# GT-RIPL/robo-vln

Measured on AMD Instinct MI355X. Metric: policy env-steps/sec (batched act()) at 256x256 RGB-D, 80-tok instr, higher is better.
Workload: dtype fp16 (range-calibrated fp16 storage and MFMA in BERT, both trunks and the cross-modal block; fp32 accumulate, fp32 recurrent state; DESIGN.md section 5); 1 GPU; BASELINE.json configs[1]: full HCM act() (hi->argmax->lo), 256x256 RGB-D, L=80, VLA N=1, LSTM-512; per_gpu_batch=64, global_batch=64, parallelism=single GPU

## Files before the change

### include/hcm.h

```cpp
#ifndef HCM_H
#define HCM_H

#include <stdint.h>

#ifdef __cplusplus
extern "C" {
#endif

typedef struct hcm_ctx* hcm_handle;

enum hcm_status {
    HCM_OK = 0,
    HCM_ERR_ARG = -1,
    HCM_ERR_STATE = -2,
    HCM_ERR_KEY = -3,
    HCM_ERR_SHAPE = -4,
    HCM_ERR_HIP = -5,
    HCM_ERR_UNSUPPORTED = -6,
    HCM_ERR_NOMEM = -7
};

enum hcm_dtype { HCM_F32 = 0, HCM_BF16 = 1, HCM_I32 = 2, HCM_I64 = 3, HCM_U8 = 4, HCM_F16 = 5 };
enum hcm_model { HCM_HIGH = 0, HCM_LOW = 1, HCM_CMA = 2 ,
                 HCM_S2S = 3  };
// ... 173 lines not shown
                  int act, void* stream);
int hcm_op_conv2d_gn(const void* x, const void* w_ohwi, const float* gamma, const float* beta, const void* residual, void* y,
                     int dtype, int B, int H, int W, int Cin, int Cout, int KH, int KW, int stride, int pad, int groups, float eps,
                     int relu, void* stream);
int hcm_op_bottleneck_tail(const void* x, const void* w2, const float* b2, const void* w3, const float* b3, const void* identity,
                           void* y, int dtype, int B, int H, int W, int C1, int stride, void* stream);
int hcm_op_bottleneck_tail_next(const void* x, const void* w2, const float* b2, const void* w3, const float* b3, const void* identity,
                                void* y, const void* w1, const float* b1, void* o1, int dtype, int B, int H, int W, int C1, int stride,
                                int CN, void* stream);
int hcm_op_bottleneck_tail_ds(const void* x, const void* w2, const float* b2, const void* w3ds, const float* b3ds, const void* xd,
                              void* y, const void* w1, const float* b1, void* o1, int dtype, int B, int H, int W, int stride,
                              void* stream);
int hcm_op_conv2d_gn_large(const void* x, const void* w_ohwi, const float* gamma, const float* beta, const void* residual, void* y,
                           int dtype, int B, int H, int W, int Cin, int Cout, int KH, int KW, int stride, int pad, int groups, float eps,
                           int relu, void* stream);
int hcm_op_stem_conv(const void* x, int x_dtype, const void* w, const float* bias, void* y, int dtype, int B, int H, int W, int C,
                     int Cout, int KH, int KW, int stride, int pad, int K, int Kp, int rowrun, float scale, int act, void* stream);
int hcm_op_stem_conv_packed(const void* x, int x_dtype, const void* w, const float* bias, void* y, int dtype, int B, int H, int W,
                            int Cout, float scale, int act, void* scratch, void* stream);
int hcm_op_stem_conv_packed_pool(const void* x, int x_dtype, const void* w, const float* bias, void* y, int dtype, int B, int H, int W,
                                 int Cout, float scale, void* scratch, void* half_map, void* stream);
int hcm_op_stem_pool_fused(const void* x, int x_dtype, const void* w, const float* bias, void* y, int dtype, int B, int H, int W,
                           int Cout, float scale, void* scratch, void* stream);
int hcm_op_stem_pool_fused_red(const void* x, int x_dtype, const void* w, const float* bias, void* y, int dtype, int B, int H, int W,
                               int Cout, float scale, void* scratch, const void* w1, const float* b1, void* o1, void* stream);
int64_t hcm_op_stem_scratch_bytes(int B, int H, int W);
int hcm_op_depth_conv8x8s4(const float* depth, const void* w, const float* bias, void* y, int dtype, int B, int H, int act, void* scratch,
                           void* stream);
int hcm_op_simplecnn3(const float* depth, const void* w0, const float* b0, const void* w1_frag, const float* b1, const void* w2_frag, const float* b2,
                      void* y, int dtype, int B, int H, void* stream);
// ... 37 lines not shown
```

### robo-vln_amd/_lib.py

```python
import ctypes as C
import os

_HERE = os.path.dirname(os.path.abspath(__file__))
LIB_PATH = os.path.join(_HERE, "libhcm_dev.so" if os.environ.get("HCM_DEV_LIB", "0") not in ("", "0") else "libhcm.so")

HCM_F32, HCM_BF16, HCM_I32, HCM_I64, HCM_U8, HCM_F16 = 0, 1, 2, 3, 4, 5
HCM_HIGH, HCM_LOW, HCM_CMA, HCM_S2S = 0, 1, 2, 3
HCM_ENC_RESNET, HCM_ENC_SIMPLECNN = 0, 1
HCM_LSTM, HCM_GRU = 0, 1
(HCM_NUM_RECURRENT_LAYERS, HCM_HIDDEN_SIZE, HCM_NUM_ACTIONS, HCM_RECORD_WIDTH, HCM_WORKSPACE_BYTES,
 HCM_WEIGHT_BYTES, HCM_MAX_BATCH, HCM_GRAPH_LAUNCHES, HCM_EAGER_LAUNCHES, HCM_FP16_FALLBACK, HCM_CALIB_MAX_BERT, HCM_CALIB_MAX_DEPTH,
 HCM_CALIB_NONFINITE, HCM_CALIB_MAX_RGB, HCM_CALIB_MAX_VLA, HCM_STEP_NONFINITE, HCM_RANGE_FOLD, HCM_GATHER_JOINED) = range(18)
PRECISIONS = {"fp32": HCM_F32, "fp16": HCM_F16, "bf16": HCM_BF16}
ACT_NONE, ACT_RELU, ACT_GELU = 0, 1, 2
HCM_ACT_REUSE_INSTRUCTION = 1
HCM_ACT_HOST_FRAMES = 2
HCM_ACT_CHAIN_GRAPHS = 4

STATUS_EXC = {-1: ValueError, -2: RuntimeError, -3: KeyError, -4: ValueError, -5: RuntimeError, -6: ValueError,
              -7: MemoryError}


class HcmConfigStruct(C.Structure):
    _fields_ = [(n, C.c_int32) for n in (
# ... 78 lines not shown
    "hcm_op_stem_pool_fused_red": (C.c_int, [C.c_void_p, C.c_int, C.c_void_p, C.c_void_p, C.c_void_p] + [C.c_int] * 5 + [C.c_float] + [C.c_void_p] * 5),
    "hcm_op_stem_conv_packed_pool": (C.c_int, [C.c_void_p, C.c_int, C.c_void_p, C.c_void_p, C.c_void_p] + [C.c_int] * 5 + [C.c_float, C.c_void_p, C.c_void_p, C.c_void_p]),
    "hcm_op_depth_conv8x8s4": (C.c_int, [C.c_void_p] * 4 + [C.c_int] * 4 + [C.c_void_p, C.c_void_p]),
    "hcm_op_stem_scratch_bytes": (C.c_int64, [C.c_int] * 3),
    "hcm_op_linear": (C.c_int, [C.c_void_p] * 5 + [C.c_int] * 6 + [C.c_void_p]),
    "hcm_op_linear_impl": (C.c_int, [C.c_void_p] * 5 + [C.c_int] * 7 + [C.c_void_p]),
    "hcm_op_vla_layer": (C.c_int, [C.c_void_p] * 7 + [C.c_int] + [C.c_void_p] * 11 + [C.c_int] * 5 + [C.c_void_p]),
    "hcm_op_vla_layer_frag": (C.c_int, [C.c_void_p] * 7 + [C.c_int] + [C.c_void_p] * 11 + [C.c_int] * 5 + [C.c_void_p]),
    "hcm_op_attention": (C.c_int, [C.c_void_p] * 4 + [C.c_int] * 9 + [C.c_void_p]),
    "hcm_op_simplecnn3": (C.c_int, [C.c_void_p] * 8 + [C.c_int] * 3 + [C.c_void_p]),
    "hcm_op_pack_frag": (C.c_int, [C.c_void_p, C.c_void_p, C.c_int, C.c_int, C.c_int, C.c_void_p]),
    "hcm_op_bert_attn_block": (C.c_int, [C.c_void_p] * 9 + [C.c_int] * 3 + [C.c_void_p, C.c_float, C.c_void_p]),
    "hcm_op_layernorm": (C.c_int, [C.c_void_p] * 5 + [C.c_int] * 3 + [C.c_float, C.c_void_p]),
    "hcm_op_layernorm_post": (C.c_int, [C.c_void_p] * 5 + [C.c_int, C.c_void_p] + [C.c_int] * 3 + [C.c_float, C.c_void_p]),
    "hcm_op_groupnorm": (C.c_int, [C.c_void_p] * 4 + [C.c_int] * 5 + [C.c_float, C.c_int, C.c_void_p]),
    "hcm_op_conv2d_gn_pool": (C.c_int, [C.c_void_p] * 5 + [C.c_int] * 11 + [C.c_float, C.c_void_p]),
    "hcm_op_conv2d_gn_res2": (C.c_int, [C.c_void_p] * 9 + [C.c_int] * 9 + [C.c_float, C.c_int, C.c_void_p]),
    "hcm_op_val_loss": (C.c_int, [C.c_void_p] * 7 + [C.c_int] * 3 + [C.c_void_p]),
    "hcm_op_maxpool3x3s2": (C.c_int, [C.c_void_p] * 2 + [C.c_int] * 5 + [C.c_void_p]),
}

_lib = None


def lib():
    global _lib
    if _lib is None:
        if not os.path.exists(LIB_PATH):
            raise RuntimeError(f"{LIB_PATH} is missing: build it with `python -c 'import __graft_entry__ as g; g.build()'` "
                               "(the HIP library is the only compute path; there is no CPU fallback)")
# ... 21 lines not shown
```

### robo-vln_amd/csrc/api.cpp

```cpp
#include <chrono>
#include <cmath>
#include <cstdlib>
#include <cstring>
#include <stdexcept>
#include <string>

#include "model.h"

namespace hcm {
void build_spec_high(hcm_ctx* ctx);
void build_spec_low(hcm_ctx* ctx);
void prepare_high(hcm_ctx* ctx);
void prepare_low(hcm_ctx* ctx);
void build_spec_cma(hcm_ctx* ctx);
void prepare_cma(hcm_ctx* ctx);
void run_refresh_instruction(hcm_ctx* ctx, const void* ids, int ids_dt, int B, const int32_t* idx, int n);
void run_cma(hcm_ctx* ctx, const void* rgb, int rgb_dt, const float* depth, const void* ids, int ids_dt, int B, const float* h_in,
             const float* mask, float* out, float* stop, float* h_out);
void build_spec_s2s(hcm_ctx* ctx);
void prepare_s2s(hcm_ctx* ctx);
void run_s2s(hcm_ctx* ctx, const void* rgb, int rgb_dt, const float* depth, const void* ids, int ids_dt, int B, int Bi, const float* h_in,
             const float* mask, float* out, float* stop, float* progress, float* h_out, int T = 1);
void comm_destroy(hcm_ctx* ctx);
void run_step(hcm_ctx* ctx, bool do_hi, bool do_lo, const void* rgb, int rgb_dt, const float* depth, const void* ids, int ids_dt,
// ... 1362 lines not shown
    if (need > scratch_floats) {
        if (scratch) { (void)hipDeviceSynchronize(); (void)hipFree(scratch); }
        if (hipMalloc((void**)&scratch, need * 4) != hipSuccess) return HCM_ERR_NOMEM;
        scratch_floats = need;
    }
    IGemm g;
    g.x = x; g.w = w_ohwi; g.y = y;
    g.B = B; g.H = H; g.W = W; g.Cin = Cin; g.xC = Cin; g.Ho = Ho; g.Wo = Wo;
    g.KH = KH; g.KW = KW; g.stride = stride; g.pad = pad;
    g.M = B * hw; g.N = Cout; g.K = KH * KW * Cin; g.Kp = g.K; g.ldy = Cout; g.ldr = Cout; g.act = ACT_NONE;
    g.cs_part = scratch; g.cs_cg = Cout / groups; g.cs_hw = hw; g.cs_G = groups;
    int rc = op_rc(launch_igemm(g, dt, (hipStream_t)stream));
    if (rc != HCM_OK) return rc;
    return op_rc(launch_groupnorm_apply(y, residual, gamma, beta, scratch, hw / 64, dt, B, hw, Cout, groups, eps, relu, (hipStream_t)stream));
}
int hcm_op_conv2d_gn_pool(const void* x, const void* w_ohwi, const float* gamma, const float* beta, void* y, int dtype, int B, int H, int W, int Cin,
                          int Cout, int KH, int KW, int stride, int pad, int groups, float eps, void* stream) {
    if (groups < 1 || Cout % groups) return HCM_ERR_ARG;
    const int Ho = (H + 2 * pad - KH) / stride + 1, Wo = (W + 2 * pad - KW) / stride + 1, hw = Ho * Wo, dt = op_dt(dtype);
    if (!groupnorm_apply_ok(dt, hw, Cout, groups) || !maxpool_gn_ok(dt, Cout, groups)) return HCM_ERR_ARG;
    const size_t stats_bytes = (gn_stats_floats(B, hw, groups) * 4 + 255) / 256 * 256, map_bytes = (size_t)B * hw * Cout * 2;
    char* sc = (char*)op_scratch(stats_bytes + map_bytes);
    if (!sc) return HCM_ERR_NOMEM;
    float* stats = (float*)sc;
    void* raw = sc + stats_bytes;
    IGemm g;
    g.x = x; g.w = w_ohwi; g.y = raw;
    g.B = B; g.H = H; g.W = W; g.Cin = Cin; g.xC = Cin; g.Ho = Ho; g.Wo = Wo;
    g.KH = KH; g.KW = KW; g.stride = stride; g.pad = pad;
    g.M = B * hw; g.N = Cout; g.K = KH * KW * Cin; g.Kp = g.K; g.ldy = Cout; g.ldr = Cout; g.act = ACT_NONE;
// ... 46 lines not shown
```

### robo-vln_amd/csrc/elementwise.hip

```cpp
#include <cstdlib>
#include "kernels.h"
#include "dev.h"

namespace hcm {

#define HCM_DISPATCH_T(dt, ...)                                           \
    do {                                                                  \
        if ((dt) == DT_BF16) { using T = bf16; __VA_ARGS__; }             \
        else if ((dt) == DT_F16) { using T = f16; __VA_ARGS__; }          \
        else if ((dt) == DT_F32) { using T = float; __VA_ARGS__; }        \
        else return hipErrorInvalidValue;                                 \
    } while (0)

static inline int grid_for(size_t n, int block = 256, int cap = 256 * 16) {
    size_t g = (n + block - 1) / block;
    if (g < 1) g = 1;
    if (g > (size_t)cap) g = cap;
    return (int)g;
}

template <typename S, typename T>
__global__ void pack_frame_kernel(const S* __restrict__ x, T* __restrict__ y, int B, int H, int W, float scale, int bt, int Hp, int Wp) {
    const size_t total = (size_t)B * Hp * Wp;
    for (size_t e = blockIdx.x * (size_t)blockDim.x + threadIdx.x; e < total; e += (size_t)gridDim.x * blockDim.x) {
// ... 584 lines not shown
    }
    int unit = Cg > CH ? Cg : CH;
    if (unit % Cg || unit % CH) {
        HCM_DISPATCH_T(dt, hipLaunchKernelGGL(gn_generic_kernel<T>, dim3(B * G), dim3(256), 0, s, (T*)x, (const T*)res, gamma, beta, HW, C, G, eps, relu, cg_true));
        return hipGetLastError();
    }
    int CS = unit;
    while (CS * 2 <= C && CS * 2 <= 256 && (CS * 2) / CH <= 32 && (long)HW * CS * 2 <= gn_slab_limit() && C % (CS * 2) == 0) CS *= 2;
    const int cpr = CS / CH;
    if (cpr & (cpr - 1) || cpr > 256 || CS > 1024 || C % CS) {
        HCM_DISPATCH_T(dt, hipLaunchKernelGGL(gn_generic_kernel<T>, dim3(B * G), dim3(256), 0, s, (T*)x, (const T*)res, gamma, beta, HW, C, G, eps, relu, cg_true));
        return hipGetLastError();
    }
    const int grid = B * (C / CS);
    HCM_DISPATCH_T(dt, hipLaunchKernelGGL(gn_fused_kernel<T>, dim3(grid), dim3(256), 0, s, (T*)x, (const T*)res, gamma, beta, HW, C, G, CS, eps, relu, cg_true));
    return hipGetLastError();
}

bool groupnorm_apply_ok(int dt, int HW, int C, int G) {
    const int CH = dt_chunk(dt);
    if (dt == DT_F32 || C % CH || C % G) return false;
    const int P = gn_partials(HW), cprw = C / CH;
    return P > 0 && !(cprw & (cprw - 1)) && cprw <= 128 && C <= 512 && G <= 256 && HW % P == 0 && HW % 64 == 0 && 32 % (C / G) == 0;
}
hipError_t launch_groupnorm_apply(void* x, const void* res, const float* gamma, const float* beta, const float* part, int PS, int dt, int B,
                                  int HW, int C, int G, float eps, int relu, hipStream_t s) {
    if (!groupnorm_apply_ok(dt, HW, C, G) || PS < 1) return hipErrorInvalidValue;
    const int P = gn_partials(HW);
    HCM_DISPATCH_T(dt, hipLaunchKernelGGL(gn_apply_kernel<T>, dim3(P, B), dim3(256), 0, s, (T*)x, (const T*)res, gamma, beta, part, HW, C, G, P, eps,
                                          relu, PS));
// ... 1004 lines not shown
```

### robo-vln_amd/csrc/forward.cpp

```cpp
#include <cstdio>
#include <cstdlib>
#include <stdexcept>

#include "model.h"

namespace hcm {

int depth_final_spatial(const hcm_config& c);
int depth_compress_channels(const hcm_config& c);

struct Act { void* p = nullptr; int B = 0, H = 0, W = 0, C = 0; };

struct Fwd {
    hcm_ctx* ctx;
    Arena& ar;
    hipStream_t s;
    int dt;
    size_t esz;
    bool dry;

    explicit Fwd(hcm_ctx* c) : ctx(c), ar(c->arena), s(c->stream), dt(c->dt_vla), esz(dt_size(c->dt_vla)), dry(c->arena.dry) {}

    void use(int d) { dt = d; esz = dt_size(d); }

// ... 23 lines not shown
            t.cap = n;
        }
        t.n = n;
        t.shape = shape;
        if (is_t) ck(launch_convert_to_f32(p, dt, t.dev, n, s), "tap convert");
        else ck(hipMemcpyAsync(t.dev, p, n * 4, hipMemcpyDeviceToDevice, s), "tap copy");
    }

    struct Pending {
        bool valid = false;
        void* x = nullptr; const void* res = nullptr; const float* stats = nullptr; const float* gamma = nullptr; const float* beta = nullptr;
        int B = 0, hw = 0, C = 0, G = 0, ps = 0, relu = 0, dt = 0; float eps = 1e-5f;
        bool writeback = false;
        const float* res_stats = nullptr; const float* res_gamma = nullptr; const float* res_beta = nullptr; float res_eps = 1e-5f;
    };
    Pending pend_in;
    Pending* defer_out = nullptr;
    Pending* res_pending = nullptr;
    void materialise_res(Pending& q) {
        if (!q.res_stats) return;
        const float* st = q.res_stats;
        q.res_stats = nullptr;
        if (dry) return;
        ck(launch_groupnorm_apply(const_cast<void*>(q.res), nullptr, q.res_gamma, q.res_beta, st, q.ps, q.dt, q.B, q.hw, q.C, q.G, q.res_eps, 0, s), "groupnorm apply (residual)");
    }
    void flush(Pending& q) {
        if (!q.valid) return;
        q.valid = false;
        if (q.res_stats) {
            const float* st = q.res_stats;
            q.res_stats = nullptr;
            if (dry) return;
            ck(launch_groupnorm_apply2(q.x, q.res, q.gamma, q.beta, q.stats, q.res_gamma, q.res_beta, st, q.ps, q.dt, q.B, q.hw, q.C, q.G, q.eps, q.res_eps, q.relu, s),
               "groupnorm apply (flush, pending residual)");
            return;
        }
        if (dry) return;
        ck(launch_groupnorm_apply(q.x, q.res, q.gamma, q.beta, q.stats, q.ps, q.dt, q.B, q.hw, q.C, q.G, q.eps, q.relu, s), "groupnorm apply (flush)");
    }
    bool gn_onload_enabled() const {
        static const bool off = dev_env("HCM_NO_GN_ONLOAD") != nullptr;
        return !off && !ctx->taps_on;
    }

    void conv_gn(const ConvW& w, const Act& in, void* out, int stride, int pad, const void* res, const NormW& n, int G, bool relu, int Ho,
                 int Wo, int cg_true = 0) {
        static const bool no_fuse = dev_env("HCM_NO_GN_FUSE") != nullptr;
        const int C = w.groups * w.Cout, cg = C / G, hw = Ho * Wo;
        struct ClearDefer { Pending*& p; ~ClearDefer() { p = nullptr; } } clear_defer{defer_out};
        Pending* rp = res_pending;
        res_pending = nullptr;
        auto settle_res = [&]() {
            if (!rp || !rp->valid) return;
            rp->valid = false;
            if (!dry) ck(launch_groupnorm_apply(rp->x, nullptr, rp->gamma, rp->beta, rp->stats, rp->ps, rp->dt, rp->B, rp->hw, rp->C, rp->G, rp->eps, rp->relu, s), "groupnorm apply (residual)");
        };
        const float eps = 1e-5f * w.fold * w.fold;
        if (cg_true) {
            settle_res();
            conv(w, in, out, stride, pad, nullptr, ACT_NONE, Ho, Wo);
            gn(out, res, n, in.B, hw, C, G, relu, cg_true, eps);
            return;
        }
        const long blocks = (long)((in.B * hw + 63) / 64) * ((w.Cout + 127) / 128) * w.groups;
        const bool fuse = !no_fuse && hw <= 64 && 64 % hw == 0 && cg % 8 == 0 && 128 % cg == 0 && w.Cout % cg == 0 && !w.bias &&
                          (blocks >= 64 || w.K < 4096);
        if (fuse) {
            settle_res();
            conv(w, in, out, stride, pad, res, relu ? ACT_RELU : ACT_NONE, Ho, Wo, &n, cg, nullptr, 0, 0, 0, eps);
        } else {
            static const bool no_cs = dev_env("HCM_NO_GN_EPISTATS") != nullptr;
            if (!no_cs && !w.bias && groupnorm_apply_ok(w.dt, hw, C, G) && w.Cout % cg == 0) {
// ... 374 lines not shown
                conv_gn(b.c3, o2, sc, 1, 0, idt, b.n3, G, true, Ho2, Wo2);
            } else {
                conv(b.c3, o2, sc, 1, 0, idt, ACT_RELU, Ho2, Wo2);
            }
            x = Act{sc, B, Ho2, Wo2, CO(b.c3)};
            xi = fr[2];
            ++bidx;
            if (bidx == 3 || bidx == 7 || bidx == 13 || bidx == 16) {
                tap(tapname + "_layer" + std::to_string(bidx == 3 ? 1 : bidx == 7 ? 2 : bidx == 13 ? 3 : 4), x.p, true, {B, x.H, x.W, x.C});
                mark(tapname + ".layer" + std::to_string(bidx == 3 ? 1 : bidx == 7 ? 2 : bidx == 13 ? 3 : 4) + "_end");
            }
        }
        flush(xpend);
        if (t.gn) {
            int fr = (xi + 1) & 3;
            conv_gn(t.compress, x, slot[fr], 1, 1, nullptr, t.n_compress, t.pair ? 2 : 1, true, x.H, x.W, t.compress_true);
            x = Act{slot[fr], B, x.H, x.W, CO(t.compress)};
        }
        dry = dry_saved;
        return x;
    }

    Act rgb_trunk(const TrunkW& t, const void* rgb, int rgb_dt, int B, const std::string& tapname) {
        const int H = ctx->cfg.rgb_h, W = ctx->cfg.rgb_w;
        const int Ho = (H + 6 - 7) / 2 + 1, Wo = (W + 6 - 7) / 2 + 1;
        calib_slot = 2;
        Act o = trunk(t, Stem{rgb, rgb_dt, 1.0f / 255.0f, H, W, 3}, B, Ho, Wo, tapname);
        calib_slot = -1;
        return o;
    }
    Act depth_trunk(const TrunkW& t, const float* depth, int B, const std::string& tapname) {
// ... 355 lines not shown
        Act o = depth_trunk(w.depth, depth, B, "hi.depth");
        void* tok = ctx->dt_depth == ctx->dt_vla ? hb.dep_tok : alloc_t((size_t)B * dS * dC);
        if (!dry) {
            ck(launch_adaptive_avgpool(o.p, tok, dt, B, o.H, o.W, o.C, o.H, o.W, dC, s), "depth tokens");
            ck(launch_fill_cols(w.depth_pe, (char*)tok + (size_t)o.C * esz, dt, B, dS, 64, dC, s), "depth pe");
            if (tok != hb.dep_tok) ck(launch_convert(tok, ctx->dt_depth, hb.dep_tok, ctx->dt_vla, (size_t)B * dS * dC, s), "depth tokens convert");
        }
        use(ctx->dt_vla);
        tap("hi.depth_spatial", hb.dep_tok, true, {B, dS, dC});
        hi_vis_pre(1, B, hb);
    }
    void depth_pair(const float* depth, int B, HiBufs& hb, LoBufs& lb) {
        const HighW& w = ctx->hi;
        const int dS = w.depth_S, dC = w.depth_C;
        use(ctx->dt_depth);
        Act o = depth_trunk(w.depth_pair, depth, B, "pair.depth");
        const int cc = o.C / 2;
        void* tok = ctx->dt_depth == ctx->dt_vla ? hb.dep_tok : alloc_t((size_t)B * dS * dC);
        void* lo_feat = alloc_t((size_t)B * dS * cc);
        if (!dry) {
            ck(launch_adaptive_avgpool(o.p, tok, dt, B, o.H, o.W, cc, o.H, o.W, dC, s, o.C), "depth tokens (hi half)");
            ck(launch_fill_cols(w.depth_pe, (char*)tok + (size_t)cc * esz, dt, B, dS, 64, dC, s), "depth pe");
            if (tok != hb.dep_tok) ck(launch_convert(tok, ctx->dt_depth, hb.dep_tok, ctx->dt_vla, (size_t)B * dS * dC, s), "depth tokens convert");
            ck(launch_adaptive_avgpool((char*)o.p + (size_t)cc * esz, lo_feat, dt, B, o.H, o.W, cc, o.H, o.W, cc, s, o.C), "depth lo half");
        }
        linear(ctx->lo.depth_fc, lo_feat, B, dS * cc, lb.xh, lb.ldx, ACT_RELU, true);
        use(ctx->dt_vla);
        tap("hi.depth_spatial", hb.dep_tok, true, {B, dS, dC});
        hi_vis_pre(1, B, hb);
    }
    void rgb_pair(const void* rgb, int rgb_dt, int B, HiBufs& hb, LoBufs& lb) {
        const HighW& w = ctx->hi;
        const hcm_config& c = ctx->cfg;
        const int rC = 2048 + 64;
        use(ctx->dt_rgb);
// ... 712 lines not shown
```

### robo-vln_amd/csrc/kernels.h

```cpp
#pragma once
#include <hip/hip_runtime.h>
#include <stdint.h>
#include <stddef.h>
#include <atomic>
#include <cstdlib>

namespace hcm {

#ifdef HCM_DEV_KNOBS
inline const char* dev_env(const char* name) { return getenv(name); }
#else
inline const char* dev_env(const char*) { return nullptr; }
#endif

struct DeviceOnce {
    std::atomic<unsigned long long> mask{0ull};
    static unsigned long long bit() { int d = 0; (void)hipGetDevice(&d); return 1ull << (d & 63); }
    bool need() const { return !(mask.load(std::memory_order_acquire) & bit()); }
    void done() { mask.fetch_or(bit(), std::memory_order_release); }
};

enum { DT_F32 = 0, DT_BF16 = 1, DT_I32 = 2, DT_I64 = 3, DT_U8 = 4, DT_F16 = 5 };
enum { ACT_NONE = 0, ACT_RELU = 1, ACT_GELU = 2 };

// ... 96 lines not shown
hipError_t launch_fill_cols(const float* tab, void* y, int dt, int B, int S, int C, int ldy, hipStream_t s);

inline int gn_partials(int HW) { return HW >= 256 ? (HW / 64 < 16 ? HW / 64 : 16) : 0; }
inline size_t gn_stats_floats(int B, int HW, int G) {
    const int P = gn_partials(HW), PS = HW % 64 == 0 ? HW / 64 : 0;
    const int n = P > PS ? P : PS;
    return (size_t)B * (n > 0 ? n : 1) * G * 2;
}
hipError_t launch_groupnorm_apply(void* x, const void* res, const float* gamma, const float* beta, const float* part, int PS, int dt, int B,
                                  int HW, int C, int G, float eps, int relu, hipStream_t s);
hipError_t launch_groupnorm_apply2(void* x, const void* res, const float* gamma, const float* beta, const float* part, const float* gamma2, const float* beta2,
                                   const float* part2, int PS, int dt, int B, int HW, int C, int G, float eps, float eps2, int relu, hipStream_t s);
bool groupnorm_apply_ok(int dt, int HW, int C, int G);
hipError_t launch_groupnorm(void* x, const void* res, const float* gamma, const float* beta, float* stats,
                            int dt, int B, int HW, int C, int G, float eps, int relu, hipStream_t s, int cg_true = 0);
hipError_t launch_layernorm(const void* x, const void* res, const float* gamma, const float* beta,
                            const float* post, int post_rows, void* y, int dt, int rows, int D, float eps, hipStream_t s);
hipError_t launch_layernorm_f32in(const float* x, const float* gamma, const float* beta, void* y16, float* y32, int dt, int rows, int D, float eps,
                                  hipStream_t s, float* stats = nullptr);
hipError_t launch_bert_embed(const void* ids, int ids_dt, const float* word, const float* pos, const float* type0,
                             const float* gamma, const float* beta, void* y, int dt, int B, int L, int D, int vocab,
                             float eps, hipStream_t s);
hipError_t launch_attention(const void* q, const void* k, const void* v, void* out, int dt, int B, int heads,
                            int Lq, int Lk, int ldq, int ldk, int ldv, int ldo, int q_batch_mod, hipStream_t s, const int* klens = nullptr);

bool bert_attn_block_ok(int dt, int D, int heads, int L, int Kp, int ldq);
hipError_t launch_pack_frag(const void* w, void* out, int dt, int N, int K, hipStream_t s);
hipError_t launch_bert_attn_block(const void* qkv, int ldq, const void* wo_frag, const float* bo, const void* res, const float* res32, const float* gamma,
                                  const float* beta, void* y, float* y32, int dt, int B, int L, const int* klens, float eps, hipStream_t s);

// ... 71 lines not shown
```

### robo-vln_amd/csrc/model.h

```cpp
#pragma once
#include <hip/hip_runtime.h>
#include <map>
#include <stdexcept>
#include <string>
#include <vector>
#include <stdint.h>

#include "../../include/hcm.h"
#include "kernels.h"

namespace hcm {

using Shape = std::vector<int64_t>;

struct HostTensor {
    std::vector<float> f;
    Shape shape;
    bool loaded = false;
};

struct ConvW {
    void* w = nullptr;
    int dt = 0;
    float* bias = nullptr;
// ... 17 lines not shown
    int stride = 1;
};
struct TrunkW {
    bool gn = false;
    bool pair = false;
    int groups = 0;
    ConvW conv1;
    ConvW conv1_rowrun;
    ConvW conv1_packed;
    int k1 = 7, s1 = 2, p1 = 3, cin1 = 3;
    NormW n_conv1;
    std::vector<BottleneckW> blocks;
    ConvW compress;
    NormW n_compress;
    int compress_true = 0;
    int out_c = 0;
};
struct SimpleCnnW {
    ConvW c0, c1, c2;
    ConvW c0_packed;
    void* c1_frag = nullptr;
    void* c2_frag = nullptr;
    LinW fc;
    int cin = 1, h = 0, w = 0, h3 = 0, w3 = 0;
};
struct BertLayerW {
    LinW qkv, o, ff1, ff2;
    void* o_frag = nullptr;
    NormW ln1, ln2;
    LinW qkv_f, ff1_f;
// ... 163 lines not shown
```

### robo-vln_amd/csrc/weights.cpp

```cpp
#include <cmath>
#include <cstdlib>
#include <cstring>
#include <stdexcept>

#include "model.h"

namespace hcm {

static const int RESNET50_BLOCKS[4] = {3, 4, 6, 3};

struct SpecB {
    std::map<std::string, HostTensor>& m;
    void add(const std::string& k, Shape s) { m[k].shape = std::move(s); }
    void conv(const std::string& k, int co, int ci, int kh, int kw) { add(k, {co, ci, kh, kw}); }
    void linear(const std::string& p, int o, int i) { add(p + ".weight", {o, i}); add(p + ".bias", {o}); }
    void norm(const std::string& p, int c) { add(p + ".weight", {c}); add(p + ".bias", {c}); }
    void bn(const std::string& p, int c) {
        norm(p, c); add(p + ".running_mean", {c}); add(p + ".running_var", {c}); add(p + ".num_batches_tracked", {});
    }
};

static void spec_tv_resnet50(SpecB& s, const std::string& pre, bool with_fc) {
    s.conv(pre + "conv1.weight", 64, 3, 7, 7); s.bn(pre + "bn1", 64);
    int inpl = 64;
// ... 402 lines not shown
    c.dt = dt;
    c.fold = fold; c.calib_pos = 0;
    const int Co = (int)ws[0]->shape[0];
    c.Cout = Co * (int)ws.size(); c.Cin = 1; c.KH = 7; c.KW = 7; c.K = 56; c.Kp = 64;
    std::vector<float> r((size_t)c.Cout * c.Kp, 0.f);
    for (size_t g = 0; g < ws.size(); ++g)
        for (int o = 0; o < Co; ++o)
            for (int kh = 0; kh < 7; ++kh)
                for (int kw = 0; kw < 7; ++kw) r[((size_t)g * Co + o) * c.Kp + kh * 8 + kw] = ws[g]->f[((size_t)o * 7 + kh) * 7 + kw] * fold;
    c.w = up.typed(r, dt);
    return c;
}

static int gn_pos(int block, int which) { return 1 + 4 * block + which; }
static float gn_fold(hcm_ctx* ctx, int pos) { return ctx->dt_depth == DT_F16 ? ctx->depth_fold[pos] : 1.f; }
static TrunkW make_gn_trunk(hcm_ctx* ctx, Uploader& up, int model, const std::string& pre) {
    TrunkW t;
    const int dt = ctx->dt_depth;
    t.gn = true;
    t.groups = ctx->cfg.depth_baseplanes / 2;
    t.cin1 = 1;
    const std::string bb = pre + "backbone.";
    auto W1 = [&](const std::string& k, int pos, int pad = 0) { return make_conv(dt, up, T_(ctx, model, k), nullptr, nullptr, pad, gn_fold(ctx, pos), pos); };
    t.conv1 = W1(bb + "conv1.0.weight", 0);
    if (dt != DT_F32) t.conv1_packed = make_depth_stem_packed(dt, up, {&T_(ctx, model, bb + "conv1.0.weight")}, gn_fold(ctx, 0));
    t.n_conv1 = make_norm(ctx, up, model, bb + "conv1.1");
    int blk = 0;
    for (int li = 0; li < 4; ++li)
        for (int bi = 0; bi < RESNET50_BLOCKS[li]; ++bi, ++blk) {
            const std::string p = bb + "layer" + std::to_string(li + 1) + "." + std::to_string(bi) + ".";
            BottleneckW b;
            b.stride = (li > 0 && bi == 0) ? 2 : 1;
            b.c1 = W1(p + "convs.0.weight", gn_pos(blk, 0)); b.n1 = make_norm(ctx, up, model, p + "convs.1");
            b.c2 = W1(p + "convs.3.weight", gn_pos(blk, 1)); b.n2 = make_norm(ctx, up, model, p + "convs.4");
            b.c3 = W1(p + "convs.6.weight", gn_pos(blk, 2)); b.n3 = make_norm(ctx, up, model, p + "convs.7");
            if (bi == 0) {
                b.has_ds = true;
                b.ds = W1(p + "downsample.0.weight", gn_pos(blk, 3));
                b.nds = make_norm(ctx, up, model, p + "downsample.1");
            }
            t.blocks.push_back(b);
        }
    const int cc = depth_compress_channels(ctx->cfg), ccp = depth_compress_padded(ctx->cfg);
    t.compress = W1(pre + "compression.0.weight", hcm_ctx::kDepthPos - 1, ccp);
    t.n_compress = make_norm(ctx, up, model, pre + "compression.1", ccp);
    t.compress_true = ccp != cc ? cc : 0;
    t.out_c = t.compress.Cout;
    return t;
}

static ConvW make_conv_pair(int dt, Uploader& up, const HostTensor& a, const HostTensor& b, bool concat_n, int cout_pad = 0, float fold = 1.f, int pos = -1) {
    ConvW c;
    c.dt = dt;
    c.fold = fold; c.calib_pos = pos;
    c.Cout = (int)a.shape[0]; c.Cin = (int)a.shape[1]; c.KH = (int)a.shape[2]; c.KW = (int)a.shape[3];
    c.K = c.KH * c.KW * c.Cin;
    c.Kp = round_up(c.K, 32);
    const int co = c.Cout;
    if (cout_pad > c.Cout) c.Cout = cout_pad;
// ... 11 lines not shown
    else c.groups = 2;
    return c;
}
static NormW make_norm_pair(hcm_ctx* ctx, Uploader& up, const std::string& p, int pad_to = 0) {
    NormW n;
    std::vector<float> g = T_(ctx, HCM_HIGH, p + ".weight").f, b = T_(ctx, HCM_HIGH, p + ".bias").f;
    std::vector<float> g2 = T_(ctx, HCM_LOW, p + ".weight").f, b2 = T_(ctx, HCM_LOW, p + ".bias").f;
    if ((int)g.size() < pad_to) { g.resize(pad_to, 0.f); b.resize(pad_to, 0.f); g2.resize(pad_to, 0.f); b2.resize(pad_to, 0.f); }
    g.insert(g.end(), g2.begin(), g2.end());
    b.insert(b.end(), b2.begin(), b2.end());
    n.C = (int)g.size();
    n.gamma = up.f32(g);
    n.beta = up.f32(b);
    return n;
}
static TrunkW make_gn_trunk_pair(hcm_ctx* ctx, Uploader& up, const std::string& pre) {
    TrunkW t;
    const int dt = ctx->dt_depth;
    t.gn = true;
    t.pair = true;
    t.groups = ctx->cfg.depth_baseplanes / 2;
    t.cin1 = 1;
    auto W2 = [&](const std::string& k, bool cat, int pos, int pad = 0) {
        return make_conv_pair(dt, up, T_(ctx, HCM_HIGH, k), T_(ctx, HCM_LOW, k), cat, pad, gn_fold(ctx, pos), pos);
    };
    const std::string bb = pre + "backbone.";
    t.conv1 = W2(bb + "conv1.0.weight", true, 0);
    if (dt != DT_F32) t.conv1_packed = make_depth_stem_packed(dt, up, {&T_(ctx, HCM_HIGH, bb + "conv1.0.weight"), &T_(ctx, HCM_LOW, bb + "conv1.0.weight")}, gn_fold(ctx, 0));
    t.n_conv1 = make_norm_pair(ctx, up, bb + "conv1.1");
    int blk = 0;
// ... 2 lines not shown
            const std::string p = bb + "layer" + std::to_string(li + 1) + "." + std::to_string(bi) + ".";
            BottleneckW b;
            b.stride = (li > 0 && bi == 0) ? 2 : 1;
            b.c1 = W2(p + "convs.0.weight", false, gn_pos(blk, 0)); b.n1 = make_norm_pair(ctx, up, p + "convs.1");
            b.c2 = W2(p + "convs.3.weight", false, gn_pos(blk, 1)); b.n2 = make_norm_pair(ctx, up, p + "convs.4");
            b.c3 = W2(p + "convs.6.weight", false, gn_pos(blk, 2)); b.n3 = make_norm_pair(ctx, up, p + "convs.7");
            if (bi == 0) {
                b.has_ds = true;
                b.ds = W2(p + "downsample.0.weight", false, gn_pos(blk, 3));
                b.nds = make_norm_pair(ctx, up, p + "downsample.1");
            }
            t.blocks.push_back(b);
        }
    const int cc = depth_compress_channels(ctx->cfg), ccp = depth_compress_padded(ctx->cfg);
    t.compress = W2(pre + "compression.0.weight", false, hcm_ctx::kDepthPos - 1, ccp);
    t.n_compress = make_norm_pair(ctx, up, pre + "compression.1", ccp);
    t.compress_true = ccp != cc ? cc : 0;
    t.out_c = t.compress.Cout;
    return t;
}

static void bn_fold(hcm_ctx* ctx, int model, const std::string& bn, int C, std::vector<float>& scale, std::vector<float>& bias, bool stem) {
    const HostTensor& g = T_(ctx, model, bn + ".weight");
    const HostTensor& b = T_(ctx, model, bn + ".bias");
    const HostTensor& m = T_(ctx, model, bn + ".running_mean");
    const HostTensor& v = T_(ctx, model, bn + ".running_var");
    const float f = ctx->dt_rgb == DT_F16 ? ctx->rgb_fold : 1.f;
    scale.resize(C); bias.resize(C);
    for (int o = 0; o < C; ++o) {
        const float s = g.f[o] / std::sqrt(v.f[o] + 1e-5f);
// ... 493 lines not shown
```

Measured before the change: 15540 env-steps/s.

## Split depth compression conv over K slices with fused groupnorm and token write

Splits the depth trunk's 3x3 compression conv into 8 input-channel slices run as extra igemm groups that write fp32 partials. A new groupnorm kernel sums the slices, normalizes them, and writes the hi-model output straight into the depth token buffer with the positional-embedding columns, and the lo-model output into the lo feature buffer. This targets low parallelism in a conv with small spatial size, large K and few output channels, and drops the separate avgpool and fill-columns launches. The cost is extra fp32 partial traffic, a fixed reduction shape limited to HW*N <= 4096, and one block per (batch, model).

```diff
diff --git a/include/hcm.h b/include/hcm.h
--- a/include/hcm.h
+++ b/include/hcm.h
@@ -211,6 +211,8 @@
 int hcm_op_conv2d_gn_large(const void* x, const void* w_ohwi, const float* gamma, const float* beta, const void* residual, void* y,
                            int dtype, int B, int H, int W, int Cin, int Cout, int KH, int KW, int stride, int pad, int groups, float eps,
                            int relu, void* stream);
+int hcm_op_conv3x3_gn_ksplit(const void* x, const void* w, const float* gamma, const float* beta, void* y, int dtype, int B, int H, int W, int Cin,
+                             int Cout, int models, float eps, int relu, int split, void* stream);
 int hcm_op_stem_conv(const void* x, int x_dtype, const void* w, const float* bias, void* y, int dtype, int B, int H, int W, int C,
                      int Cout, int KH, int KW, int stride, int pad, int K, int Kp, int rowrun, float scale, int act, void* stream);
 int hcm_op_stem_conv_packed(const void* x, int x_dtype, const void* w, const float* bias, void* y, int dtype, int B, int H, int W,
diff --git a/robo-vln_amd/_lib.py b/robo-vln_amd/_lib.py
--- a/robo-vln_amd/_lib.py
+++ b/robo-vln_amd/_lib.py
@@ -116,6 +116,7 @@
     "hcm_op_layernorm": (C.c_int, [C.c_void_p] * 5 + [C.c_int] * 3 + [C.c_float, C.c_void_p]),
     "hcm_op_layernorm_post": (C.c_int, [C.c_void_p] * 5 + [C.c_int, C.c_void_p] + [C.c_int] * 3 + [C.c_float, C.c_void_p]),
     "hcm_op_groupnorm": (C.c_int, [C.c_void_p] * 4 + [C.c_int] * 5 + [C.c_float, C.c_int, C.c_void_p]),
+    "hcm_op_conv3x3_gn_ksplit": (C.c_int, [C.c_void_p] * 5 + [C.c_int] * 7 + [C.c_float, C.c_int, C.c_int, C.c_void_p]),
     "hcm_op_conv2d_gn_pool": (C.c_int, [C.c_void_p] * 5 + [C.c_int] * 11 + [C.c_float, C.c_void_p]),
     "hcm_op_conv2d_gn_res2": (C.c_int, [C.c_void_p] * 9 + [C.c_int] * 9 + [C.c_float, C.c_int, C.c_void_p]),
     "hcm_op_val_loss": (C.c_int, [C.c_void_p] * 7 + [C.c_int] * 3 + [C.c_void_p]),
diff --git a/robo-vln_amd/csrc/api.cpp b/robo-vln_amd/csrc/api.cpp
--- a/robo-vln_amd/csrc/api.cpp
+++ b/robo-vln_amd/csrc/api.cpp
@@ -1400,6 +1400,35 @@
     if (rc != HCM_OK) return rc;
     return op_rc(launch_groupnorm_apply(y, residual, gamma, beta, scratch, hw / 64, dt, B, hw, Cout, groups, eps, relu, (hipStream_t)stream));
 }
+int hcm_op_conv3x3_gn_ksplit(const void* x, const void* w, const float* gamma, const float* beta, void* y, int dtype, int B, int H, int W, int Cin,
+                             int Cout, int models, float eps, int relu, int split, void* stream) {
+    const int dt = op_dt(dtype), hw = H * W, M = B * hw;
+    constexpr int S = 8;
+    if (models < 1 || B < 1 || hw < 1) return HCM_ERR_ARG;
+    IGemm g;
+    g.x = x; g.w = w;
+    g.B = B; g.H = H; g.W = W; g.xC = models * Cin; g.Ho = H; g.Wo = W; g.KH = 3; g.KW = 3; g.stride = 1; g.pad = 1;
+    g.M = M; g.N = Cout; g.act = ACT_NONE;
+    if (!split) {
+        g.y = y; g.Cin = Cin; g.K = g.Kp = 9 * Cin; g.ldy = g.ldr = models * Cout;
+        g.groups = models; g.g_x = Cin; g.g_w = (long long)Cout * g.Kp; g.g_b = Cout; g.g_y = Cout;
+        const int rc = op_rc(launch_igemm(g, dt, (hipStream_t)stream));
+        if (rc != HCM_OK) return rc;
+        return op_rc(launch_groupnorm(y, nullptr, gamma, beta, nullptr, dt, B, hw, models * Cout, models, eps, relu, (hipStream_t)stream));
+    }
+    if (Cin % (S * 64) || !groupnorm_ksplit_ok(dt, hw, Cout, S)) return HCM_ERR_ARG;
+    float* part = (float*)op_scratch((size_t)models * S * M * Cout * 4);
+    if (!part) return HCM_ERR_NOMEM;
+    const int Cs = Cin / S;
+    g.y = part; g.Cin = Cs; g.K = g.Kp = 9 * Cs; g.ldy = g.ldr = Cout; g.out_f32 = 1;
+    g.groups = models * S; g.g_x = Cs; g.g_w = (long long)Cout * g.Kp; g.g_b = 0; g.g_y = (long long)M * Cout;
+    const int rc = op_rc(launch_igemm(g, dt, (hipStream_t)stream));
+    if (rc != HCM_OK) return rc;
+    if (models > 2) return HCM_ERR_ARG;
+    GnKsplitOut o;
+    for (int m = 0; m < models; ++m) { o.y[m] = (char*)y + (size_t)m * Cout * 2; o.ld[m] = models * Cout; }
+    return op_rc(launch_groupnorm_ksplit(part, o, gamma, beta, dt, B, hw, Cout, models, S, eps, relu, 0, (hipStream_t)stream));
+}
 int hcm_op_conv2d_gn_pool(const void* x, const void* w_ohwi, const float* gamma, const float* beta, void* y, int dtype, int B, int H, int W, int Cin,
                           int Cout, int KH, int KW, int stride, int pad, int groups, float eps, void* stream) {
     if (groups < 1 || Cout % groups) return HCM_ERR_ARG;
diff --git a/robo-vln_amd/csrc/elementwise.hip b/robo-vln_amd/csrc/elementwise.hip
--- a/robo-vln_amd/csrc/elementwise.hip
+++ b/robo-vln_amd/csrc/elementwise.hip
@@ -622,6 +622,79 @@
     }
     const int grid = B * (C / CS);
     HCM_DISPATCH_T(dt, hipLaunchKernelGGL(gn_fused_kernel<T>, dim3(grid), dim3(256), 0, s, (T*)x, (const T*)res, gamma, beta, HW, C, G, CS, eps, relu, cg_true));
+    return hipGetLastError();
+}
+
+template <typename T, int S>
+__global__ __launch_bounds__(256) void gn_ksplit_kernel(const float* __restrict__ part, GnKsplitOut out, const float* __restrict__ gamma,
+                                                         const float* __restrict__ beta, int HW, int N, int G, long long slice, float eps, int relu,
+                                                         int cg_true) {
+    __shared__ float s_red[2][4];
+    const int b = blockIdx.x / G, g = blockIdx.x % G;
+    const int tid = threadIdx.x;
+    const int n4 = HW * N / 4;
+    const float* pb = part + (size_t)g * S * slice + (size_t)b * HW * N;
+    const int ldy = g ? out.ld[1] : out.ld[0];
+    T* yb = (T*)(g ? out.y[1] : out.y[0]) + (size_t)b * HW * ldy;
+    float4 v[4];
+    float s1 = 0.f, s2 = 0.f;
+#pragma unroll
+    for (int it = 0; it < 4; ++it) {
+        const int i = tid + it * 256;
+        float4 a = make_float4(0.f, 0.f, 0.f, 0.f);
+        if (i < n4) {
+            a = *reinterpret_cast<const float4*>(pb + (size_t)i * 4);
+#pragma unroll
+            for (int sl = 1; sl < S; ++sl) {
+                const float4 q = *reinterpret_cast<const float4*>(pb + (size_t)sl * slice + (size_t)i * 4);
+                a.x += q.x; a.y += q.y; a.z += q.z; a.w += q.w;
+            }
+        }
+        v[it] = a;
+        s1 += (a.x + a.y) + (a.z + a.w);
+        s2 += (a.x * a.x + a.y * a.y) + (a.z * a.z + a.w * a.w);
+    }
+    for (int o = 32; o >= 1; o >>= 1) { s1 += __shfl_xor(s1, o, 64); s2 += __shfl_xor(s2, o, 64); }
+    if ((tid & 63) == 0) { s_red[0][tid >> 6] = s1; s_red[1][tid >> 6] = s2; }
+    __syncthreads();
+    const float a = (s_red[0][0] + s_red[0][1]) + (s_red[0][2] + s_red[0][3]);
+    const float q = (s_red[1][0] + s_red[1][1]) + (s_red[1][2] + s_red[1][3]);
+    const float inv_n = 1.0f / ((float)HW * (float)(cg_true > 0 ? cg_true : N));
+    const float mean = a * inv_n;
+    const float rstd = rsqrtf(relu_f(q * inv_n - mean * mean) + eps);
+#pragma unroll
+    for (int it = 0; it < 4; ++it) {
+        const int i = tid + it * 256;
+        if (i >= n4) continue;
+        const int e = i * 4, p = e / N, c = e % N;
+        const float4 ga = *reinterpret_cast<const float4*>(gamma + g * N + c);
+        const float4 be = *reinterpret_cast<const float4*>(beta + g * N + c);
+        float o[4] = {(v[it].x - mean) * rstd * ga.x + be.x, (v[it].y - mean) * rstd * ga.y + be.y, (v[it].z - mean) * rstd * ga.z + be.z,
+                      (v[it].w - mean) * rstd * ga.w + be.w};
+        T t[4];
+#pragma unroll
+        for (int j = 0; j < 4; ++j) Tr<T>::st(&t[j], relu ? relu_f(o[j]) : o[j]);
+        *reinterpret_cast<uint2*>(yb + (size_t)p * ldy + c) = *reinterpret_cast<const uint2*>(t);
+    }
+    if (g == 0 && out.pe) {
+        for (int i = tid; i < HW * out.pe_cols; i += 256) {
+            const int p = i / out.pe_cols, c = i % out.pe_cols;
+            Tr<T>::st(yb + (size_t)p * ldy + N + c, out.pe[i]);
+        }
+    }
+}
+bool groupnorm_ksplit_ok(int dt, int HW, int N, int S) {
+    return (dt == DT_F16 || dt == DT_BF16) && S == 8 && HW >= 1 && N >= 4 && N % 4 == 0 && (long)HW * N <= 4096;
+}
+hipError_t launch_groupnorm_ksplit(const float* part, const GnKsplitOut& out, const float* gamma, const float* beta, int dt, int B, int HW, int N, int G, int S,
+                                   float eps, int relu, int cg_true, hipStream_t s) {
+    if (!groupnorm_ksplit_ok(dt, HW, N, S) || B < 1 || G < 1 || G > 2 || cg_true < 0 || cg_true > N) return hipErrorInvalidValue;
+    for (int g = 0; g < G; ++g)
+        if (!out.y[g] || out.ld[g] < N || out.ld[g] % 4 || ((size_t)out.y[g] & 7)) return hipErrorInvalidValue;
+    if (out.pe && (out.pe_cols < 1 || out.ld[0] < N + out.pe_cols)) return hipErrorInvalidValue;
+    const long long slice = (long long)B * HW * N;
+    if (dt == DT_F16) hipLaunchKernelGGL((gn_ksplit_kernel<f16, 8>), dim3(B * G), dim3(256), 0, s, part, out, gamma, beta, HW, N, G, slice, eps, relu, cg_true);
+    else hipLaunchKernelGGL((gn_ksplit_kernel<bf16, 8>), dim3(B * G), dim3(256), 0, s, part, out, gamma, beta, HW, N, G, slice, eps, relu, cg_true);
     return hipGetLastError();
 }
 
diff --git a/robo-vln_amd/csrc/forward.cpp b/robo-vln_amd/csrc/forward.cpp
--- a/robo-vln_amd/csrc/forward.cpp
+++ b/robo-vln_amd/csrc/forward.cpp
@@ -61,6 +61,8 @@
         bool writeback = false;
         const float* res_stats = nullptr; const float* res_gamma = nullptr; const float* res_beta = nullptr; float res_eps = 1e-5f;
     };
+    const GnKsplitOut* ks_out = nullptr;
+    bool ks_out_taken = false;
     Pending pend_in;
     Pending* defer_out = nullptr;
     Pending* res_pending = nullptr;
@@ -91,7 +93,7 @@
     }
 
     void conv_gn(const ConvW& w, const Act& in, void* out, int stride, int pad, const void* res, const NormW& n, int G, bool relu, int Ho,
-                 int Wo, int cg_true = 0) {
+                 int Wo, int cg_true = 0, const ConvW* wks = nullptr) {
         static const bool no_fuse = dev_env("HCM_NO_GN_FUSE") != nullptr;
         const int C = w.groups * w.Cout, cg = C / G, hw = Ho * Wo;
         struct ClearDefer { Pending*& p; ~ClearDefer() { p = nullptr; } } clear_defer{defer_out};
@@ -103,6 +105,30 @@
             if (!dry) ck(launch_groupnorm_apply(rp->x, nullptr, rp->gamma, rp->beta, rp->stats, rp->ps, rp->dt, rp->B, rp->hw, rp->C, rp->G, rp->eps, rp->relu, s), "groupnorm apply (residual)");
         };
         const float eps = 1e-5f * w.fold * w.fold;
+        static const bool no_ks = dev_env("HCM_NO_CONV_KSPLIT") != nullptr;
+        if (wks && wks->w && !no_ks && !res && !rp && !pend_in.valid && stride == 1 && pad == 1 && !w.bias && w.KH == 3 && w.KW == 3 && G == w.groups &&
+            G <= 2 && wks->groups == w.groups * TrunkW::kCompressSlices && wks->Cout == w.Cout && wks->Cin * TrunkW::kCompressSlices == w.Cin &&
+            in.C == w.groups * w.Cin && wks->dt == w.dt && groupnorm_ksplit_ok(w.dt, hw, w.Cout, TrunkW::kCompressSlices)) {
+            const int M = in.B * hw;
+            float* part = alloc_f((size_t)wks->groups * M * w.Cout);
+            if (ks_out) ks_out_taken = true;
+            if (dry) return;
+            IGemm g;
+            g.x = in.p; g.w = wks->w; g.y = part;
+            g.B = in.B; g.H = in.H; g.W = in.W; g.Cin = wks->Cin; g.xC = in.C;
+            g.Ho = Ho; g.Wo = Wo; g.KH = 3; g.KW = 3; g.stride = 1; g.pad = 1;
+            g.M = M; g.N = w.Cout; g.K = wks->K; g.Kp = wks->Kp; g.ldy = g.ldr = w.Cout; g.act = ACT_NONE; g.out_f32 = 1;
+            g.groups = wks->groups; g.g_x = wks->Cin; g.g_w = (long long)w.Cout * wks->Kp; g.g_b = 0; g.g_y = (long long)M * w.Cout;
+            static const int ks_choice = dev_env("HCM_KS_CHOICE") ? atoi(dev_env("HCM_KS_CHOICE")) : 15;
+            g.force_choice = ks_choice;
+            ck(launch_igemm(g, w.dt, s), "conv igemm (K slices)");
+            GnKsplitOut o;
+            if (ks_out) o = *ks_out;
+            else for (int gi = 0; gi < 2 && gi < G; ++gi) { o.y[gi] = (char*)out + (size_t)gi * w.Cout * dt_size(w.dt); o.ld[gi] = C; }
+            ck(launch_groupnorm_ksplit(part, o, n.gamma, n.beta, w.dt, in.B, hw, w.Cout, G, TrunkW::kCompressSlices, eps, relu ? 1 : 0, cg_true, s),
+               "groupnorm over K slices");
+            return;
+        }
         if (cg_true) {
             settle_res();
             conv(w, in, out, stride, pad, nullptr, ACT_NONE, Ho, Wo);
@@ -507,7 +533,7 @@
         flush(xpend);
         if (t.gn) {
             int fr = (xi + 1) & 3;
-            conv_gn(t.compress, x, slot[fr], 1, 1, nullptr, t.n_compress, t.pair ? 2 : 1, true, x.H, x.W, t.compress_true);
+            conv_gn(t.compress, x, slot[fr], 1, 1, nullptr, t.n_compress, t.pair ? 2 : 1, true, x.H, x.W, t.compress_true, &t.compress_ks);
             x = Act{slot[fr], B, x.H, x.W, CO(t.compress)};
         }
         dry = dry_saved;
@@ -893,11 +919,20 @@
         const HighW& w = ctx->hi;
         const int dS = w.depth_S, dC = w.depth_C;
         use(ctx->dt_depth);
-        Act o = depth_trunk(w.depth_pair, depth, B, "pair.depth");
-        const int cc = o.C / 2;
+        static const bool no_direct = dev_env("HCM_NO_KS_DIRECT") != nullptr;
+        const int cc = w.depth_pair.compress.Cout;
         void* tok = ctx->dt_depth == ctx->dt_vla ? hb.dep_tok : alloc_t((size_t)B * dS * dC);
         void* lo_feat = alloc_t((size_t)B * dS * cc);
-        if (!dry) {
+        GnKsplitOut ko;
+        ko.y[0] = tok; ko.ld[0] = dC; ko.y[1] = lo_feat; ko.ld[1] = cc; ko.pe = w.depth_pe; ko.pe_cols = 64;
+        ks_out_taken = false;
+        if (!no_direct && !ctx->taps_on && dC >= cc + 64) ks_out = &ko;
+        Act o = depth_trunk(w.depth_pair, depth, B, "pair.depth");
+        ks_out = nullptr;
+        if (o.C != 2 * cc || o.H * o.W != dS) throw std::runtime_error("depth pair trunk: unexpected output shape");
+        if (ks_out_taken) {
+            if (!dry && tok != hb.dep_tok) ck(launch_convert(tok, ctx->dt_depth, hb.dep_tok, ctx->dt_vla, (size_t)B * dS * dC, s), "depth tokens convert");
+        } else if (!dry) {
             ck(launch_adaptive_avgpool(o.p, tok, dt, B, o.H, o.W, cc, o.H, o.W, dC, s, o.C), "depth tokens (hi half)");
             ck(launch_fill_cols(w.depth_pe, (char*)tok + (size_t)cc * esz, dt, B, dS, 64, dC, s), "depth pe");
             if (tok != hb.dep_tok) ck(launch_convert(tok, ctx->dt_depth, hb.dep_tok, ctx->dt_vla, (size_t)B * dS * dC, s), "depth tokens convert");
diff --git a/robo-vln_amd/csrc/kernels.h b/robo-vln_amd/csrc/kernels.h
--- a/robo-vln_amd/csrc/kernels.h
+++ b/robo-vln_amd/csrc/kernels.h
@@ -134,6 +134,15 @@
 bool groupnorm_apply_ok(int dt, int HW, int C, int G);
 hipError_t launch_groupnorm(void* x, const void* res, const float* gamma, const float* beta, float* stats,
                             int dt, int B, int HW, int C, int G, float eps, int relu, hipStream_t s, int cg_true = 0);
+struct GnKsplitOut {
+    void* y[2] = {nullptr, nullptr};
+    int ld[2] = {0, 0};
+    const float* pe = nullptr;
+    int pe_cols = 0;
+};
+bool groupnorm_ksplit_ok(int dt, int HW, int N, int S);
+hipError_t launch_groupnorm_ksplit(const float* part, const GnKsplitOut& out, const float* gamma, const float* beta, int dt, int B, int HW, int N, int G, int S,
+                                   float eps, int relu, int cg_true, hipStream_t s);
 hipError_t launch_layernorm(const void* x, const void* res, const float* gamma, const float* beta,
                             const float* post, int post_rows, void* y, int dt, int rows, int D, float eps, hipStream_t s);
 hipError_t launch_layernorm_f32in(const float* x, const float* gamma, const float* beta, void* y16, float* y32, int dt, int rows, int D, float eps,
diff --git a/robo-vln_amd/csrc/model.h b/robo-vln_amd/csrc/model.h
--- a/robo-vln_amd/csrc/model.h
+++ b/robo-vln_amd/csrc/model.h
@@ -55,6 +55,8 @@
     ConvW compress;
     NormW n_compress;
     int compress_true = 0;
+    ConvW compress_ks;
+    static constexpr int kCompressSlices = 8;
     int out_c = 0;
 };
 struct SimpleCnnW {
diff --git a/robo-vln_amd/csrc/weights.cpp b/robo-vln_amd/csrc/weights.cpp
--- a/robo-vln_amd/csrc/weights.cpp
+++ b/robo-vln_amd/csrc/weights.cpp
@@ -440,6 +440,7 @@
 
 static int gn_pos(int block, int which) { return 1 + 4 * block + which; }
 static float gn_fold(hcm_ctx* ctx, int pos) { return ctx->dt_depth == DT_F16 ? ctx->depth_fold[pos] : 1.f; }
+static ConvW make_conv_kslices(int dt, Uploader& up, const std::vector<const HostTensor*>& ws, int cout_pad, float fold);
 static TrunkW make_gn_trunk(hcm_ctx* ctx, Uploader& up, int model, const std::string& pre) {
     TrunkW t;
     const int dt = ctx->dt_depth;
@@ -469,6 +470,7 @@
         }
     const int cc = depth_compress_channels(ctx->cfg), ccp = depth_compress_padded(ctx->cfg);
     t.compress = W1(pre + "compression.0.weight", hcm_ctx::kDepthPos - 1, ccp);
+    t.compress_ks = make_conv_kslices(dt, up, {&T_(ctx, model, pre + "compression.0.weight")}, ccp, gn_fold(ctx, hcm_ctx::kDepthPos - 1));
     t.n_compress = make_norm(ctx, up, model, pre + "compression.1", ccp);
     t.compress_true = ccp != cc ? cc : 0;
     t.out_c = t.compress.Cout;
@@ -510,6 +512,29 @@
     n.beta = up.f32(b);
     return n;
 }
+static ConvW make_conv_kslices(int dt, Uploader& up, const std::vector<const HostTensor*>& ws, int cout_pad, float fold) {
+    ConvW c;
+    const HostTensor& a = *ws[0];
+    constexpr int S = TrunkW::kCompressSlices;
+    const int Cin = (int)a.shape[1];
+    if ((dt != DT_F16 && dt != DT_BF16) || a.shape[2] != 3 || a.shape[3] != 3 || Cin % (S * 64) || ((Cin / S) & (Cin / S - 1))) return c;
+    c.dt = dt;
+    c.fold = fold;
+    const int co = (int)a.shape[0], Cs = Cin / S;
+    c.Cout = cout_pad > co ? cout_pad : co; c.Cin = Cs; c.KH = 3; c.KW = 3;
+    c.K = c.Kp = 9 * Cs;
+    c.groups = (int)ws.size() * S;
+    std::vector<float> r((size_t)c.groups * c.Cout * c.Kp, 0.f);
+    for (size_t g = 0; g < ws.size(); ++g)
+        for (int s = 0; s < S; ++s)
+            for (int o = 0; o < co; ++o)
+                for (int i = 0; i < Cs; ++i)
+                    for (int t = 0; t < 9; ++t)
+                        r[((g * S + s) * c.Cout + o) * c.Kp + (size_t)t * Cs + i] = ws[g]->f[((size_t)o * Cin + s * Cs + i) * 9 + t] * fold;
+    c.w = up.typed(r, dt);
+    return c;
+}
+
 static TrunkW make_gn_trunk_pair(hcm_ctx* ctx, Uploader& up, const std::string& pre) {
     TrunkW t;
     const int dt = ctx->dt_depth;
@@ -542,6 +567,8 @@
         }
     const int cc = depth_compress_channels(ctx->cfg), ccp = depth_compress_padded(ctx->cfg);
     t.compress = W2(pre + "compression.0.weight", false, hcm_ctx::kDepthPos - 1, ccp);
+    t.compress_ks = make_conv_kslices(dt, up, {&T_(ctx, HCM_HIGH, pre + "compression.0.weight"), &T_(ctx, HCM_LOW, pre + "compression.0.weight")}, ccp,
+                                      gn_fold(ctx, hcm_ctx::kDepthPos - 1));
     t.n_compress = make_norm_pair(ctx, up, pre + "compression.1", ccp);
     t.compress_true = ccp != cc ? cc : 0;
     t.out_c = t.compress.Cout;
```

Result: no change. 15480 env-steps/s (-0.4%).
